# tensorlayer/HyperPose

Hardware: NVIDIA H100
Metric: frames/sec end-to-end (conv+PAF parse) OpenPose-COCO 368x656 (higher is better)
Workload: dtype f16 operands, f32 accumulate (conv); f32/f64 (parse)

## Files before the change

### hyperpose_b200/capi.py

```python
from __future__ import annotations

import ctypes as C
import os
import struct

import numpy as np

PKG = os.path.dirname(os.path.abspath(__file__))
LIB_PATH = os.path.join(PKG, "libhyperpose_b200.so")

N_PARTS, N_PAIRS = 18, 19
HP_OK, HP_ERR_ARG, HP_ERR_CAPACITY, HP_ERR_UNSUPPORTED, HP_ERR_CUDA, HP_ERR_BATCH = 0, -1, -2, -3, -4, -5

PART_DT = np.dtype({"names": ["has_value", "x", "y", "score"], "formats": ["<i4", "<f4", "<f4", "<f4"]})
HUMAN_DT = np.dtype([("parts", PART_DT, (N_PARTS,)), ("score", "<f4")])
PEAK_DT = np.dtype([("part_id", "<i4"), ("x", "<i4"), ("y", "<i4"), ("score", "<f4"), ("id", "<i4")])
CONN_DT = np.dtype([("cid1", "<i4"), ("cid2", "<i4"), ("score", "<f4")])
assert HUMAN_DT.itemsize == 292

EXPORTS = [
    "hp_last_error", "hp_device_count", "hp_version",
    "hp_paf_create", "hp_paf_destroy", "hp_paf_set_conf_thresh", "hp_paf_set_paf_thresh", "hp_paf_set_capacity",
    "hp_paf_process_host", "hp_paf_process_host_batched", "hp_paf_process_device", "hp_paf_fetch",
    "hp_paf_debug_peaks", "hp_paf_debug_connections", "hp_paf_launch_count", "hp_paf_copy_results_device", "hp_paf_debug_timing",
# ... 151 lines not shown
        _bind_engine(L)
        L._engine_bound = True
    check(L.hp_handoff_enable(1 if on else 0))


EXPORTS += [
    "hp_engine_create", "hp_engine_destroy", "hp_engine_info", "hp_engine_infer_u8_host", "hp_engine_infer_u8_device",
    "hp_engine_infer_f32_host", "hp_engine_outputs", "hp_engine_read_outputs_host", "hp_engine_copy_outputs_device", "hp_engine_sync",
    "hp_engine_launch_count", "hp_engine_debug_read_buffer", "hp_engine_debug_write_buffer", "hp_engine_debug_run_ops",
    "hp_pose_run_u8_host", "hp_engine_stage_frame_u8", "hp_engine_infer_staged", "hp_engine_debug_read_frames", "hp_engine_set_output_override", "hp_engine_set_profiling", "hp_engine_get_profile",
    "hp_engine_read_outputs_frames", "hp_engine_head_type", "hp_handoff_enable", "hp_handoff_stats",
    "hp_pose_submit_u8_host", "hp_pose_collect", "hp_pose_stats", "hp_paf_prepare", "hp_paf_state", "hp_paf_copy_results_host_async",
    "hp_paf_grow_capacity", "hp_pool_create", "hp_pool_destroy", "hp_pool_size", "hp_pool_set_capacity", "hp_pool_run_u8_host",
    "hp_pool_set_output_override", "hp_pool_launch_count", "hp_default_device", "hp_handoff_device_of",
    "hp_engine_create_ex", "hp_engine_dtype", "hp_pose_submit_u8_device", "hp_engine_debug_op_kernel",
    "hp_engine_debug_op_epilogue",
    "hp_engine_calibrate_u8", "hp_pack_int8_calibrated",
]


def _bind_engine(L):
    vp, ip = C.c_void_p, C.POINTER(C.c_int)
    L.hp_engine_create.argtypes = [C.POINTER(vp), vp, C.c_size_t, C.c_int, C.c_int, C.c_int, C.c_double, C.c_int, C.c_int]
    L.hp_engine_create_ex.argtypes = [C.POINTER(vp), vp, C.c_size_t, C.c_int, C.c_int, C.c_int, C.c_double, C.c_int, C.c_int, C.c_int]
    L.hp_engine_dtype.argtypes = [vp]
    L.hp_engine_destroy.argtypes = [vp]
    L.hp_engine_destroy.restype = None
    L.hp_engine_info.argtypes = [vp, ip, ip, ip, ip, ip, ip, ip, C.POINTER(C.c_double)]
    L.hp_engine_infer_u8_host.argtypes = [vp, vp, C.c_int]
    L.hp_engine_infer_u8_device.argtypes = [vp, vp, C.c_int, vp]
    L.hp_engine_infer_f32_host.argtypes = [vp, vp, C.c_int]
    L.hp_engine_outputs.argtypes = [vp, C.POINTER(vp), C.POINTER(vp), C.POINTER(vp)]
    L.hp_engine_read_outputs_host.argtypes = [vp, vp, vp, C.c_int]
    L.hp_engine_sync.argtypes = [vp]
    L.hp_engine_copy_outputs_device.argtypes = [vp, vp, vp, C.c_int, vp]
    L.hp_engine_launch_count.argtypes = [vp]
    L.hp_engine_launch_count.restype = C.c_longlong
    L.hp_engine_debug_read_buffer.argtypes = [vp, C.c_int, vp, C.c_int, ip, ip, ip]
    L.hp_engine_debug_write_buffer.argtypes = [vp, C.c_int, vp, C.c_int]
    L.hp_engine_debug_run_ops.argtypes = [vp, C.c_int, C.c_int, C.c_int]
    L.hp_engine_debug_op_kernel.argtypes = [vp, C.c_int, C.c_char_p, C.c_int]
    L.hp_engine_debug_op_epilogue.argtypes = [vp, C.c_int, ip]
    L.hp_engine_calibrate_u8.argtypes = [vp, vp, C.c_int, vp, C.c_int]
    L.hp_pack_int8_calibrated.argtypes = [vp, C.c_size_t]
    L.hp_pose_run_u8_host.argtypes = [vp, vp, vp, C.c_int, vp, C.c_int, ip]
    L.hp_engine_stage_frame_u8.argtypes = [vp, C.c_int, vp, C.c_int, C.c_int, C.c_int]
    L.hp_engine_infer_staged.argtypes = [vp, C.c_int]
    L.hp_engine_debug_read_frames.argtypes = [vp, vp, C.c_int]
    L.hp_engine_set_output_override.argtypes = [vp, vp, vp]
    L.hp_engine_set_profiling.argtypes = [vp, C.c_int]
    L.hp_engine_get_profile.argtypes = [vp, vp, vp, vp, C.c_int, ip, C.POINTER(C.c_longlong)]
    L.hp_engine_read_outputs_frames.argtypes = [vp, C.POINTER(vp), C.POINTER(vp), C.c_int, C.c_int]
    L.hp_engine_head_type.argtypes = [vp]
    L.hp_handoff_enable.argtypes = [C.c_int]
    L.hp_handoff_stats.argtypes = [C.POINTER(C.c_longlong)] * 4
    L.hp_pose_submit_u8_host.argtypes = [vp, vp, vp, C.c_int, ip]
    L.hp_pose_submit_u8_device.argtypes = [vp, vp, vp, C.c_int, ip]
# ... 143 lines not shown
        return out

    def debug_run_ops(self, first: int, last: int, n: int):
        check(lib().hp_engine_debug_run_ops(self._h, first, last, n))

    def debug_op_kernel(self, op: int) -> str:
        buf = C.create_string_buffer(64)
        check(lib().hp_engine_debug_op_kernel(self._h, op, buf, len(buf)))
        return buf.value.decode()

    def debug_op_epilogue(self, op: int) -> str:
        v = C.c_int(0)
        check(lib().hp_engine_debug_op_epilogue(self._h, op, C.byref(v)))
        return "tma" if v.value else "reg"

    def set_output_override(self, d_conf_ptr: int, d_paf_ptr: int):
        check(lib().hp_engine_set_output_override(self._h, d_conf_ptr, d_paf_ptr))

    def set_profiling(self, enable: bool):
        check(lib().hp_engine_set_profiling(self._h, 1 if enable else 0))

    def get_profile(self):
        cap = 1024
        ms = np.zeros(cap, np.float64); ty = np.zeros(cap, np.int32); fl = np.zeros(cap, np.float64)
        n, runs = C.c_int(), C.c_longlong()
        check(lib().hp_engine_get_profile(self._h, ms.ctypes.data, ty.ctypes.data, fl.ctypes.data, cap, C.byref(n), C.byref(runs)))
        return ms[:n.value], ty[:n.value], fl[:n.value], runs.value

    def run_pose(self, parser: "PafParser", frames: np.ndarray, cap: int = 128):
        frames = np.ascontiguousarray(frames, np.uint8)
# ... 242 lines not shown
```

### hyperpose_b200/csrc/conv_wgmma.cuh

```cuda
#pragma once
#include <cuda.h>
#include <cuda_fp16.h>
#include <cuda_runtime.h>
#include <stdint.h>

#include <type_traits>

namespace hpb {

constexpr int CONV_BLOCK_M = 128;
constexpr int CONV_BLOCK_K = 64;
constexpr int TF32_BLOCK_K = 32;
constexpr int CONV_MAX_STAGES = 8;
constexpr int CONV_THREADS = 384;
constexpr int CONV_A_BYTES = CONV_BLOCK_M * 128;
constexpr size_t CONV_SMEM_LIMIT = 227 * 1024;

enum ConvOutMode : int {
    OUT_F16_NHWC = 0,
    OUT_F32_NCHW_SPLIT = 1,
};

struct ConvParams {
    int Nb, H, W;
// ... 694 lines not shown
__device__ __forceinline__ uint64_t make_sw128_kmajor_desc_at(uint32_t smem_addr, uint32_t sbo)
{
    uint64_t d = 0;
    d |= (uint64_t)((smem_addr & 0x3ffffu) >> 4);
    d |= (uint64_t)1 << 16;
    d |= (uint64_t)((sbo >> 4) & 0x3fffu) << 32;
    d |= (uint64_t)1 << 62;
    return d;
}
template <uint32_t N> __device__ __forceinline__ void setmaxnreg_dec() { asm volatile("setmaxnreg.dec.sync.aligned.u32 %0;" ::"n"(N)); }
template <uint32_t N> __device__ __forceinline__ void setmaxnreg_inc() { asm volatile("setmaxnreg.inc.sync.aligned.u32 %0;" ::"n"(N)); }
__device__ __forceinline__ void stmatrix_x4(uint32_t addr, uint32_t r0, uint32_t r1, uint32_t r2, uint32_t r3)
{
    asm volatile("stmatrix.sync.aligned.m8n8.x4.shared.b16 [%0], {%1, %2, %3, %4};" ::"r"(addr), "r"(r0), "r"(r1), "r"(r2), "r"(r3) : "memory");
}
__device__ __forceinline__ void st_shared_u32(uint32_t addr, uint32_t v) { asm volatile("st.shared.b32 [%0], %1;" ::"r"(addr), "r"(v) : "memory"); }
__device__ __forceinline__ void named_barrier_sync(int id, int threads) { asm volatile("bar.sync %0, %1;" ::"r"(id), "r"(threads) : "memory"); }
__device__ __forceinline__ void tma_store_4d(const CUtensorMap* m, uint32_t src, int c0, int c1, int c2, int c3)
{
    asm volatile("cp.async.bulk.tensor.4d.global.shared::cta.bulk_group [%0, {%2, %3, %4, %5}], [%1];"
                 ::"l"(m), "r"(src), "r"(c0), "r"(c1), "r"(c2), "r"(c3) : "memory");
}
__device__ __forceinline__ void bulk_commit() { asm volatile("cp.async.bulk.commit_group;" ::: "memory"); }
template <int N> __device__ __forceinline__ void bulk_wait_read() { asm volatile("cp.async.bulk.wait_group.read %0;" ::"n"(N) : "memory"); }
template <int N> __device__ __forceinline__ void bulk_wait() { asm volatile("cp.async.bulk.wait_group %0;" ::"n"(N) : "memory"); }
__device__ __forceinline__ uint32_t half2_bits(__half2 h) { return *reinterpret_cast<uint32_t*>(&h); }
}

template <int BN, bool kPool, int kBlocks>
__device__ __forceinline__ void halo_epilogue(const float (&acc)[kBlocks][BN / 2], const HaloParams& p, int n, int y0, int x0, int g, int n0,
                                              int row_base, int warp, int lane)
// ... 119 lines not shown
                }
            }
        }
        ptx::fence_proxy_async();
        ptx::named_barrier_sync(bar_id, 128);
        if (leader) {
            const int x = kPool ? x0 >> 1 : x0, y = kPool ? (y0 + ty0) >> 1 : y0 + ty0;
            ptx::tma_store_4d(tmap_o, slot, och, x, y, n);
            if (BN == 128 && n0 + 64 < p.cout_g)
                ptx::tma_store_4d(tmap_o, slot + (uint32_t)kSliceBytes, och + 64, x, y, n);
            ptx::bulk_commit();
        }
    }
}

template <int BN, int kBlocks>
__device__ __forceinline__ void halo_kstep(float (&acc)[kBlocks][BN / 2], uint32_t abase, int r, int s, int BW, uint32_t sbo, const uint8_t* s_b,
                                           uint64_t* b_full, RingPos b, int c_or_tap HALO_PH_PARAM)
{
    uint64_t da[kBlocks];
#pragma unroll
    for (int m = 0; m < kBlocks; ++m) da[m] = ptx::make_sw128_kmajor_desc_at(abase + (uint32_t)(((m * 8 + r) * BW + s) * 128), sbo);
    const uint64_t db = ptx::make_sw128_kmajor_desc(ptx::smem_u32(s_b + (size_t)b.slot * BN * 128));
    HALO_TIMED(HALO_PH_B_WAIT, ptx::mbar_wait(ptx::smem_u32(b_full + b.slot), b.phase));
#pragma unroll
    for (int m = 0; m < kBlocks; ++m) ptx::fence_acc(acc[m]);
    ptx::wgmma_fence();
#pragma unroll
    for (int k = 0; k < 4; ++k)
#pragma unroll
// ... 14 lines not shown
        if (tma) {
            if constexpr (kItem != HaloItem::Wide)
                halo_epilogue_tma<BN, kPool, kShape.blocks, kShape.stage_slots, true>(acc, p, tmap_o, stage, n, y0, x0, g, n0, row_base, warp, lane,
                                                                                     leader HALO_PH_ARG);
            else if (p.box_bytes >= kShape.blocks * BN * 128)
                halo_epilogue_tma<BN, kPool, kShape.blocks, kShape.blocks, false>(acc, p, tmap_o, stage, n, y0, x0, g, n0, row_base, warp, lane,
                                                                                 leader HALO_PH_ARG);
            else
                halo_epilogue_tma<BN, kPool, kShape.blocks, 1, true>(acc, p, tmap_o, stage, n, y0, x0, g, n0, row_base, warp, lane, leader HALO_PH_ARG);
            return;
        }
    }
    halo_epilogue<BN, kPool, kShape.blocks>(acc, p, n, y0, x0, g, n0, row_base, warp, lane);
}

template <int BN, bool kPool, HaloItem kItem>
__global__ void __launch_bounds__(CONV_THREADS, 1)
conv_halo_kernel(const __grid_constant__ CUtensorMap tmap_x, const __grid_constant__ CUtensorMap tmap_b, const __grid_constant__ CUtensorMap tmap_o,
                 const HaloParams p)
{
    static_assert(!(kItem == HaloItem::Wide && kPool), "the pooled epilogue pairs pixel rows of one m64 block; it has no wide form");
    static_assert(kItem != HaloItem::PingPong || BN == 64 || BN == 128, "the ping-pong item is built for the VGG trunk's widths, BN = 64 and 128");
    constexpr HaloShape kShape = halo_shape(kItem, BN);
    constexpr int B_BYTES = BN * 128;
    constexpr bool kTmaForm = BN % 64 == 0;
    extern __shared__ uint8_t smem_raw[];
    ptx::pdl_launch_dependents();
    uint8_t* smem = (uint8_t*)(((uintptr_t)smem_raw + 1023) & ~(uintptr_t)1023);
    uint8_t* s_box = smem;
    uint8_t* s_b = s_box + (size_t)kShape.box_slots * kShape.tiles * p.box_bytes;
    uint8_t* s_stage = s_b + (size_t)p.num_stages * B_BYTES;
    uint64_t* a_full = (uint64_t*)(s_stage + 2 * (size_t)p.stage_bytes);
    uint64_t* a_empty = a_full + kShape.box_slots;
    uint64_t* b_full = a_empty + kShape.box_slots;
    uint64_t* b_empty = b_full + CONV_MAX_STAGES;
    uint64_t* turn = b_empty + CONV_MAX_STAGES;

    const int wg = threadIdx.x >> 7, warp = threadIdx.x >> 5, lane = threadIdx.x & 31;
    const int n_tiles_g = p.cout_g_pad / BN;
    const int nt_total = p.groups * n_tiles_g;
    const int sp_per_img = p.tiles_x * p.tiles_y;
    const int total_items = (p.Nb * sp_per_img + kShape.tiles - 1) / kShape.tiles * nt_total;
    const int chunks = p.cin_g / CONV_BLOCK_K;
    const int taps = p.R * p.S;
    const int BW = HALO_TW + p.S - 1, BH = HALO_TH + p.R - 1;

    if (threadIdx.x == 0) {
        ptx::prefetch_tmap(&tmap_x);
        ptx::prefetch_tmap(&tmap_b);
        if (kTmaForm && p.tma_store) ptx::prefetch_tmap(&tmap_o);
        for (int i = 0; i < kShape.box_slots; ++i) {
            ptx::mbar_init(ptx::smem_u32(a_full + i), 1);
            ptx::mbar_init(ptx::smem_u32(a_empty + i), kShape.slot_warps);
        }
        for (int i = 0; i < p.num_stages; ++i) {
            ptx::mbar_init(ptx::smem_u32(b_full + i), 1);
            ptx::mbar_init(ptx::smem_u32(b_empty + i), kShape.slot_warps);
        }
        if constexpr (kItem == HaloItem::PingPong) {
            ptx::mbar_init(ptx::smem_u32(turn), 4);
            ptx::mbar_init(ptx::smem_u32(turn + 1), 4);
        }
        ptx::fence_barrier_init();
    }
    __syncthreads();
    ptx::pdl_wait();

    auto decode = [&](int item, int& sp, int& g, int& n0) {
        const int nt = item % nt_total;
        sp = item / nt_total * kShape.tiles;
        g = nt / n_tiles_g;
        n0 = (nt - g * n_tiles_g) * BN;
    };
    auto tile_pos = [&](int sp, int& n, int& y0, int& x0) {
        n = sp / sp_per_img;
        const int t = sp - n * sp_per_img;
        const int ty = t / p.tiles_x;
        y0 = ty * HALO_TH;
// ... 11 lines not shown
            const int pad_h = p.R / 2, pad_w = p.S / 2;
            for (int item = blockIdx.x; item < total_items; item += gridDim.x) {
                int sp, g, n0;
                decode(item, sp, g, n0);
                for (int c = 0; c < chunks; ++c) {
                    ptx::mbar_wait(ptx::smem_u32(a_empty + a.slot), a.phase ^ 1);
                    const uint32_t fa = ptx::smem_u32(a_full + a.slot);
                    ptx::mbar_expect_tx(fa, (uint32_t)(kShape.tiles * BH * BW * 128));
#pragma unroll
                    for (int t = 0; t < kShape.tiles; ++t) {
                        int n, y0, x0;
                        tile_pos(sp + t, n, y0, x0);
                        ptx::tma_load_4d(ptx::smem_u32(s_box + (size_t)(a.slot * kShape.tiles + t) * p.box_bytes), &tmap_x, fa,
                                         p.in_ch_off + g * p.cin_g + c * CONV_BLOCK_K, x0 - pad_w, y0 - pad_h, n);
                    }
                    a.step(kShape.box_slots);
                    for (int tap = 0; tap < taps; ++tap) {
                        ptx::mbar_wait(ptx::smem_u32(b_empty + b.slot), b.phase ^ 1);
                        const uint32_t fb = ptx::smem_u32(b_full + b.slot);
                        ptx::mbar_expect_tx(fb, (uint32_t)B_BYTES);
                        ptx::tma_load_2d(ptx::smem_u32(s_b + (size_t)b.slot * B_BYTES), &tmap_b, fb, tap * p.cin_g + c * CONV_BLOCK_K, g * p.cout_g_pad + n0);
                        b.step(p.num_stages);
                    }
                }
            }
        }
        return;
    }

    if constexpr (kShape.move_regs) ptx::setmaxnreg_inc<HALO_WIDE_CONSUMER_REGS>();
    const int half = wg - 1;
    const uint32_t sbo = (uint32_t)BW * 128u;
    const bool tma = kTmaForm && p.tma_store;
    const bool leader = (threadIdx.x & 127) == 0;
    const uint32_t stage = ptx::smem_u32(s_stage + (size_t)half * p.stage_bytes);
    float acc[kShape.blocks][BN / 2];
    if constexpr (kItem == HaloItem::PingPong) {
        const int item_stages = chunks * taps;
        if (half) {
            a.advance(chunks, kShape.box_slots);
            b.advance(item_stages, p.num_stages);
        }
        for (int j = half, item = blockIdx.x + half * gridDim.x; item < total_items; j += 2, item += 2 * gridDim.x) {
            int sp, g, n0;
            decode(item, sp, g, n0);
            if (j > 0) HALO_TIMED(HALO_PH_TURN_WAIT, ptx::mbar_wait(ptx::smem_u32(turn + half), (uint32_t)((j - 1) >> 1) & 1u));
            int prev_st = 0, prev_bs = 0;
            for (int c = 0; c < chunks; ++c) {
                HALO_TIMED(HALO_PH_A_WAIT, ptx::mbar_wait(ptx::smem_u32(a_full + a.slot), a.phase));
                const uint32_t abase = ptx::smem_u32(s_box + (size_t)a.slot * p.box_bytes);
                for (int tap = 0; tap < taps; ++tap) {
                    const int r = tap / p.S, s = tap - r * p.S;
// ... 74 lines not shown
            const int last = (a.slot + kShape.box_slots - 1) % kShape.box_slots;
            const uint32_t dst = kItem == HaloItem::Wide ? ptx::smem_u32(s_box + (size_t)(last * kShape.tiles + box) * p.box_bytes) : stage;
            halo_store<BN, kPool, kItem>(acc, p, &tmap_o, tma, dst, n, y0, x0, g, n0, row_base, warp, lane, leader HALO_PH_ARG);
            HALO_PH_ADD(HALO_PH_EPILOGUE, t_epi);
        }
    }
    if (tma && leader) ptx::bulk_wait<0>();
#ifdef HPB_HALO_PHASES
    HALO_PH_ADD(HALO_PH_TOTAL, t_start);
    if ((threadIdx.x & 127) == 0)
        for (int i = 0; i < HALO_PH_COUNT; ++i) atomicAdd(g_halo_phases + i, (unsigned long long)ph[i]);
#endif
}

inline int halo_box_bytes(int R, int S) { return ((HALO_TH + R - 1) * (HALO_TW + S - 1) * 128 + 1023) & ~1023; }
inline size_t conv_halo_smem_bytes(int R, int S, int BN, int stages, HaloItem it, bool tma_store)
{
    const HaloShape sh = halo_shape(it, BN);
    return 1024 + (size_t)sh.box_slots * sh.tiles * halo_box_bytes(R, S) + (size_t)stages * BN * 128 +
           (tma_store ? 2 * (size_t)halo_stage_bytes(BN, it) : 0) + (2 * sh.box_slots + 2 * CONV_MAX_STAGES + 2) * 8;
}
inline int conv_halo_pick_stages(int R, int S, int BN, HaloItem it, bool tma_store)
{
    int s = CONV_MAX_STAGES;
    while (s > 2 && conv_halo_smem_bytes(R, S, BN, s, it, tma_store) > CONV_SMEM_LIMIT) --s;
    return s;
}

}
```

### hyperpose_b200/csrc/engine.cu

```cuda
#include <cuda.h>
#include <cuda_fp16.h>
#include <cuda_runtime.h>
#include <math.h>
#include <stdint.h>
#include <stdlib.h>
#include <string.h>

#include <algorithm>
#include <memory>
#include <string>
#include <vector>

#include "../../include/hyperpose_b200.h"
#include "common.h"
#include "conv_wgmma.cuh"
#include "helpers_tf32_int8.cuh"
#include "handoff.h"
#include "pair_math.cuh"
#include "pack_format.h"

namespace {
using namespace hpb;


// ... 506 lines not shown
    for (int bn : { 96, 64 })
        if (round_up(cout_g, bn) < round_up(cout_g, best)) best = bn;
    return best;
}

struct ConvPlan {
    ConvParams prm;
    CUtensorMap tmap_a, tmap_b;
    CUtensorMap tmap_x;
    CUtensorMap tmap_o;
    void* d_w = nullptr;
    bool monotone_act = false;
    HaloParams hp;
    HaloItem halo_item = HaloItem::Narrow;
    bool halo_pool = false;
    float* d_bias = nullptr;
    float* d_alpha = nullptr;
    float* d_mul = nullptr;
    size_t smem = 0;
    double flops_per_frame = 0;
};

enum class Launch : uint8_t {
    None,
    Im2col,
    StemOrIm2col,
    Conv,
    ConvStem,
    Halo,
    DwTma,
// ... 132 lines not shown
inline float tf32_round(float x)
{
    uint32_t u;
    memcpy(&u, &x, 4);
    if ((u & 0x7f800000u) != 0x7f800000u) u = (u + 0x1000u) & 0xffffe000u;
    memcpy(&x, &u, 4);
    return x;
}

bool halo_tma_store_ok(const HaloParams& h, int BN)
{
    return BN % 64 == 0 && h.out_ld % 8 == 0 && h.out_ch_off % 8 == 0 && (h.groups * h.cout_g) % 8 == 0 &&
           (h.groups == 1 || h.cout_g % BN == 0);
}

int set_halo_item(const hp_engine* e, EngOp& op, HaloItem item, bool pool)
{
    HaloParams& h = op.plan.hp;
    const int BN = op.plan.prm.BN;
    h.tma_store = e->opt.halo_tma_store && halo_tma_store_ok(h, BN);
    h.stage_bytes = h.tma_store ? halo_stage_bytes(BN, item) : 0;
    h.num_stages = conv_halo_pick_stages(h.R, h.S, BN, item, h.tma_store);
    op.plan.smem = conv_halo_smem_bytes(h.R, h.S, BN, h.num_stages, item, h.tma_store);
    op.plan.halo_item = item;
    op.plan.halo_pool = pool;
    op.launch = Launch::Halo;
    if (!h.tma_store) return HP_OK;
    const int oh = pool ? h.H / 2 : h.H, ow = pool ? h.W / 2 : h.W, box = pool ? HALO_TW / 2 : HALO_TW;
    return make_tmap_act_box(&op.plan.tmap_o, h.out, e->max_batch, oh, ow, h.out_ch_off + h.groups * h.cout_g, h.out_ld, box, box,
                             CU_TENSOR_MAP_SWIZZLE_128B);
}

bool halo_wide_faster(int R, long wide_items, int sms)
{
    return R == 7 && wide_items >= sms;
}

bool halo_pp_exists(int R, int BN) { return R == 3 && (BN == 64 || BN == 128); }
bool halo_pp_faster(int chunks, bool pooled, long items, int sms) { return (chunks >= 4 || pooled) && items >= 2L * sms; }
// ... 174 lines not shown
}

template <typename T, bool kRes, int kStemR = 0>
const void* conv_kernel_bn(int BN)
{
    switch (BN) {
    case 16: return (const void*)conv_wgmma_kernel<T, 16, kRes, kStemR>;
    case 32: return (const void*)conv_wgmma_kernel<T, 32, kRes, kStemR>;
    case 48: return (const void*)conv_wgmma_kernel<T, 48, kRes, kStemR>;
    case 64: return (const void*)conv_wgmma_kernel<T, 64, kRes, kStemR>;
    case 96: return (const void*)conv_wgmma_kernel<T, 96, kRes, kStemR>;
    case 128: return (const void*)conv_wgmma_kernel<T, 128, kRes, kStemR>;
    }
    return nullptr;
}
const void* halo_kernel(int BN, HaloItem item, bool pool)
{
    using I = HaloItem;
    if (item == I::Wide) return BN == 128 && !pool ? (const void*)conv_halo_kernel<128, false, I::Wide> : nullptr;
    if (item == I::PingPong) {
        if (BN == 64) return pool ? (const void*)conv_halo_kernel<64, true, I::PingPong> : (const void*)conv_halo_kernel<64, false, I::PingPong>;
        if (BN == 128) return pool ? (const void*)conv_halo_kernel<128, true, I::PingPong> : (const void*)conv_halo_kernel<128, false, I::PingPong>;
        return nullptr;
    }
    switch (BN) {
    case 16: return pool ? (const void*)conv_halo_kernel<16, true, I::Narrow> : (const void*)conv_halo_kernel<16, false, I::Narrow>;
    case 32: return pool ? (const void*)conv_halo_kernel<32, true, I::Narrow> : (const void*)conv_halo_kernel<32, false, I::Narrow>;
    case 48: return pool ? (const void*)conv_halo_kernel<48, true, I::Narrow> : (const void*)conv_halo_kernel<48, false, I::Narrow>;
    case 64: return pool ? (const void*)conv_halo_kernel<64, true, I::Narrow> : (const void*)conv_halo_kernel<64, false, I::Narrow>;
    case 96: return pool ? (const void*)conv_halo_kernel<96, true, I::Narrow> : (const void*)conv_halo_kernel<96, false, I::Narrow>;
    case 128: return pool ? (const void*)conv_halo_kernel<128, true, I::Narrow> : (const void*)conv_halo_kernel<128, false, I::Narrow>;
    }
    return nullptr;
}
// ... 28 lines not shown
int launch_conv(hp_engine* e, EngOp& op, int N, cudaStream_t st, bool u8_input)
{
    ConvPlan& pl = op.plan;
    ConvParams p = pl.prm;
    p.Nb = N;
    const int stem_R = op.launch == Launch::ConvStem && u8_input ? (int)op.po.R : 0;
    p.frames = e->cur_frames ? e->cur_frames : e->d_frames;
    if (op.launch == Launch::Halo) {
        HaloParams h = pl.hp;
        h.Nb = N;
        const int tiles = halo_shape(pl.halo_item, p.BN).tiles;
        const long items = ((long)N * h.tiles_x * h.tiles_y + tiles - 1) / tiles * h.groups * (h.cout_g_pad / p.BN);
        cudaLaunchAttribute at[1];
        const cudaLaunchConfig_t cfg = pdl_config((int)std::min<long>(e->num_sms - e->reserve_sms, items), CONV_THREADS, pl.smem, st, at);
        void* args[] = { (void*)&pl.tmap_x, (void*)&pl.tmap_b, (void*)&pl.tmap_o, (void*)&h };
        HP_CUDA_TRY(cudaLaunchKernelExC(&cfg, halo_kernel(p.BN, pl.halo_item, pl.halo_pool), args));
        return HP_OK;
    }
    p.m_tiles = (int)(((size_t)N * p.H * p.W + CONV_BLOCK_M - 1) / CONV_BLOCK_M);
    const int n_tiles = p.m_tiles * p.groups * (p.cout_g_pad / p.BN);
    const int grid = std::min(e->num_sms - e->reserve_sms, n_tiles);
    cudaLaunchAttribute at[1];
    const cudaLaunchConfig_t cfg = pdl_config(grid, CONV_THREADS, pl.smem, st, at);
    void* args[] = { (void*)&pl.tmap_a, (void*)&pl.tmap_b, (void*)&p };
    HP_CUDA_TRY(cudaLaunchKernelExC(&cfg, conv_kernel(e->dtype, p.res_mode != 0, p.BN, stem_R), args));
    return HP_OK;
}

bool collect_one(hp_engine* e, bool blocking)
{
    if (e->ev_tail >= e->ev_head) return false;
// ... 569 lines not shown
        if (a.launch != Launch::DwTma || b.launch != Launch::DwTma || a.po.in_buf != b.po.in_buf || a.po.in_ch_off != b.po.in_ch_off ||
            a.po.cout_g != b.po.cout_g || a.po.out_buf != b.po.out_buf || dw_dilation(a.po) != 1 || dw_dilation(b.po) != 1) continue;
        a.launch = Launch::DwTmaPair;
        b.launch = Launch::None;
    }
    int launches = 0;
    for (const EngOp& o : e->ops) {
        if ((o.po.type == OP_CONV || o.po.type == OP_DWCONV || o.po.type == OP_MAXPOOL2) && o.launch != Launch::None) ++launches;
        e->step_kernels += kernels_launched(o.launch, true);
    }
    const double per_launch = launches ? e->flops_per_frame * e->max_batch / launches : 0.0;
    e->use_pdl = dtype == HP_DTYPE_F16 && launches > 0 && per_launch < 10e9;
    for (const EngOp& o : e->ops) {
        if (o.po.type != OP_CONV) continue;
        if (o.launch == Launch::Halo &&
            cudaFuncSetAttribute(halo_kernel(o.plan.prm.BN, o.plan.halo_item, o.plan.halo_pool), cudaFuncAttributeMaxDynamicSharedMemorySize, (int)max_smem) != cudaSuccess) {
            set_error("engine: cannot opt in to %zu bytes of dynamic shared memory (halo)", max_smem);
            return fail(HP_ERR_CUDA);
        }
        const int stem_R = o.launch == Launch::ConvStem ? (int)o.po.R : 0;
        for (int v = 0; v < 3; ++v)
            if ((v < 2 || stem_R) &&
                cudaFuncSetAttribute(conv_kernel(dtype, v == 1, o.plan.prm.BN, v == 2 ? stem_R : 0), cudaFuncAttributeMaxDynamicSharedMemorySize, (int)max_smem) != cudaSuccess) {
                set_error("engine: cannot opt in to %zu bytes of dynamic shared memory", max_smem);
                return fail(HP_ERR_CUDA);
            }
    }
    if (cudaDeviceSynchronize() != cudaSuccess) { set_error("hp_engine_create: device error during set-up: %s", cudaGetErrorString(cudaGetLastError())); return fail(HP_ERR_CUDA); }
    *out = e;
    return HP_OK;
}
// ... 341 lines not shown
        s = s.back() == '>' ? s.substr(0, s.size() - 1) + "," + d + ">" : s + "<" + d + ">";
    }
    if ((int)s.size() >= cap) { set_error("hp_engine_debug_op_kernel: %zu-character name, capacity %d", s.size(), cap); return HP_ERR_CAPACITY; }
    memcpy(name, s.c_str(), s.size() + 1);
    return HP_OK;
}

int hp_engine_debug_op_epilogue(const hp_engine* e, int op, int* tma_store)
{
    if (!e || op < 0 || op >= (int)e->ops.size() || !tma_store) { set_error("hp_engine_debug_op_epilogue: bad argument"); return HP_ERR_ARG; }
    const EngOp& o = e->ops[op];
    *tma_store = o.launch == Launch::Halo && o.plan.hp.tma_store ? 1 : 0;
    return HP_OK;
}

long long hp_engine_launch_count(const hp_engine* e) { return e ? e->launches : 0; }

int hp_engine_set_output_override(hp_engine* e, const float* d_conf, const float* d_paf)
{
    if (!e) return HP_ERR_ARG;
    e->override_conf = d_conf;
    e->override_paf = d_paf;
    return HP_OK;
}

int hp_engine_set_profiling(hp_engine* e, int enable)
{
    if (!e) return HP_ERR_ARG;
    HP_CUDA_TRY(cudaSetDevice(e->device));
    if (enable && e->ev.empty()) {
// ... 326 lines not shown
```

### include/hyperpose_b200.h

```cpp
#ifndef HYPERPOSE_B200_H
#define HYPERPOSE_B200_H

#include <stddef.h>
#include <stdint.h>

#ifdef __cplusplus
extern "C" {
#endif

#define HP_N_PARTS 18
#define HP_N_PAIRS 19

typedef enum hp_status {
    HP_OK = 0,
    HP_ERR_ARG = -1,
    HP_ERR_CAPACITY = -2,
    HP_ERR_UNSUPPORTED = -3,
    HP_ERR_CUDA = -4,
    HP_ERR_BATCH = -5
} hp_status;

typedef struct hp_body_part {
    int32_t has_value;
    float x, y, score;
// ... 90 lines not shown
int hp_engine_infer_f32_host(hp_engine* e, const float* nchw, int N);
int hp_engine_outputs(hp_engine* e, const float** d_conf, const float** d_paf, void** stream);
int hp_engine_read_outputs_host(hp_engine* e, float* conf, float* paf, int N);
int hp_engine_read_outputs_frames(hp_engine* e, float* const* conf_frames, float* const* paf_frames, int N, int publish);
int hp_engine_head_type(const hp_engine* e);
int hp_handoff_enable(int on);
int hp_handoff_stats(long long* published, long long* hits, long long* batch_parses, long long* misses);
int hp_engine_copy_outputs_device(hp_engine* e, float* d_conf, float* d_paf, int N, void* stream);
int hp_engine_sync(hp_engine* e);
long long hp_engine_launch_count(const hp_engine* e);
int hp_engine_debug_read_buffer(hp_engine* e, int buf, void* out_f16, int N, int* H, int* W, int* C);
int hp_engine_debug_write_buffer(hp_engine* e, int buf, const void* in_f16, int N);
int hp_engine_debug_run_ops(hp_engine* e, int first_op, int last_op, int N);
int hp_engine_debug_op_kernel(const hp_engine* e, int op, char* name, int cap);
int hp_engine_debug_op_epilogue(const hp_engine* e, int op, int* tma_store);

int hp_engine_set_output_override(hp_engine* e, const float* d_conf, const float* d_paf);
int hp_engine_set_profiling(hp_engine* e, int enable);
int hp_engine_get_profile(hp_engine* e, double* ms_per_op, int* op_type, double* flops_per_op, int cap, int* n_ops, long long* runs);

int hp_pose_run_u8_host(hp_engine* e, hp_paf* parser, const uint8_t* frames, int N, hp_human* out, int cap, int* n_out);
int hp_pose_submit_u8_host(hp_engine* e, hp_paf* parser, const uint8_t* frames, int N, int* ticket);
int hp_pose_submit_u8_device(hp_engine* e, hp_paf* parser, const uint8_t* d_frames, int N, int* ticket);
int hp_pose_collect(hp_engine* e, int ticket, hp_human* out, int cap, int* n_out);
int hp_pose_stats(const hp_engine* e, long long* graph_captures, long long* graph_launches);
int hp_pose_submit_pifpaf_u8_host(hp_engine* e, hp_pifpaf* decoder, const uint8_t* frames, int N, int* ticket);
int hp_pose_submit_pifpaf_u8_device(hp_engine* e, hp_pifpaf* decoder, const uint8_t* d_frames, int N, int* ticket);
int hp_pifpaf_pipeline_info(hp_pifpaf* p, void** stream, void** inputs_free_event, int* hcap);
int hp_pifpaf_copy_results_host_async(hp_pifpaf* p, hp_human* pin_humans, int* pin_counts_flags, int N, void* stream);
int hp_pifpaf_grow_capacity(hp_pifpaf* p, int flags);
// ... 22 lines not shown
```

Baseline: 1024.

## Keep 3x3 conv weights resident in shared memory for the 64-channel ping-pong halo kernel

For 3x3, 64-in/64-out, ungrouped convs using the ping-pong halo item, all nine weight tap tiles are loaded into shared memory once per CTA. The per-item B-tile streaming loop and its full/empty barriers are removed, and the freed smem is spent on extra input box slots. The MMA computes with weights as the A operand, giving a channel-major accumulator. A new epilogue writes it with transposed stmatrix (or a pooled u16 scatter) before the TMA store. This cuts redundant weight TMA traffic and producer synchronisation on the early VGG layers, at the cost of a new epilogue layout path that may be less efficient or carry indexing bugs.

Measured after the change: 1055 (median of 6 runs). 3.0% higher.

```diff
diff --git a/hyperpose_b200/capi.py b/hyperpose_b200/capi.py
--- a/hyperpose_b200/capi.py
+++ b/hyperpose_b200/capi.py
@@ -189,7 +189,7 @@
     "hp_paf_grow_capacity", "hp_pool_create", "hp_pool_destroy", "hp_pool_size", "hp_pool_set_capacity", "hp_pool_run_u8_host",
     "hp_pool_set_output_override", "hp_pool_launch_count", "hp_default_device", "hp_handoff_device_of",
     "hp_engine_create_ex", "hp_engine_dtype", "hp_pose_submit_u8_device", "hp_engine_debug_op_kernel",
-    "hp_engine_debug_op_epilogue",
+    "hp_engine_debug_op_epilogue", "hp_engine_debug_op_weights",
     "hp_engine_calibrate_u8", "hp_pack_int8_calibrated",
 ]
 
@@ -216,6 +216,7 @@
     L.hp_engine_debug_run_ops.argtypes = [vp, C.c_int, C.c_int, C.c_int]
     L.hp_engine_debug_op_kernel.argtypes = [vp, C.c_int, C.c_char_p, C.c_int]
     L.hp_engine_debug_op_epilogue.argtypes = [vp, C.c_int, ip]
+    L.hp_engine_debug_op_weights.argtypes = [vp, C.c_int, ip]
     L.hp_engine_calibrate_u8.argtypes = [vp, vp, C.c_int, vp, C.c_int]
     L.hp_pack_int8_calibrated.argtypes = [vp, C.c_size_t]
     L.hp_pose_run_u8_host.argtypes = [vp, vp, vp, C.c_int, vp, C.c_int, ip]
@@ -389,6 +390,11 @@
         check(lib().hp_engine_debug_op_epilogue(self._h, op, C.byref(v)))
         return "tma" if v.value else "reg"
 
+    def debug_op_weights(self, op: int) -> str:
+        v = C.c_int(0)
+        check(lib().hp_engine_debug_op_weights(self._h, op, C.byref(v)))
+        return "resident" if v.value else "streamed"
+
     def set_output_override(self, d_conf_ptr: int, d_paf_ptr: int):
         check(lib().hp_engine_set_output_override(self._h, d_conf_ptr, d_paf_ptr))
 
diff --git a/hyperpose_b200/csrc/conv_wgmma.cuh b/hyperpose_b200/csrc/conv_wgmma.cuh
--- a/hyperpose_b200/csrc/conv_wgmma.cuh
+++ b/hyperpose_b200/csrc/conv_wgmma.cuh
@@ -732,7 +732,12 @@
 {
     asm volatile("stmatrix.sync.aligned.m8n8.x4.shared.b16 [%0], {%1, %2, %3, %4};" ::"r"(addr), "r"(r0), "r"(r1), "r"(r2), "r"(r3) : "memory");
 }
+__device__ __forceinline__ void stmatrix_x4_trans(uint32_t addr, uint32_t r0, uint32_t r1, uint32_t r2, uint32_t r3)
+{
+    asm volatile("stmatrix.sync.aligned.m8n8.x4.trans.shared.b16 [%0], {%1, %2, %3, %4};" ::"r"(addr), "r"(r0), "r"(r1), "r"(r2), "r"(r3) : "memory");
+}
 __device__ __forceinline__ void st_shared_u32(uint32_t addr, uint32_t v) { asm volatile("st.shared.b32 [%0], %1;" ::"r"(addr), "r"(v) : "memory"); }
+__device__ __forceinline__ void st_shared_u16(uint32_t addr, unsigned short v) { asm volatile("st.shared.b16 [%0], %1;" ::"r"(addr), "h"(v) : "memory"); }
 __device__ __forceinline__ void named_barrier_sync(int id, int threads) { asm volatile("bar.sync %0, %1;" ::"r"(id), "r"(threads) : "memory"); }
 __device__ __forceinline__ void tma_store_4d(const CUtensorMap* m, uint32_t src, int c0, int c1, int c2, int c3)
 {
@@ -882,6 +887,63 @@
     }
 }
 
+template <bool kPool>
+__device__ __forceinline__ void halo_epilogue_tma_cm(const float (&acc)[64], const HaloParams& p, const CUtensorMap* tmap_o, uint32_t stage,
+                                                     int n, int y0, int x0, int warp, int lane, bool leader HALO_PH_PARAM)
+{
+    constexpr int kSliceBytes = (kPool ? 16 : 64) * 128;
+    const int c = 16 * (warp & 3) + (lane >> 2);
+    const float b[2] = { __ldg(p.bias + c), __ldg(p.bias + c + 8) }, a[2] = { __ldg(p.alpha + c), __ldg(p.alpha + c + 8) };
+    const int bar_id = warp >> 2;
+#pragma unroll
+    for (int m = 0; m < 2; ++m) {
+        const uint32_t slot = stage + (uint32_t)(m * kSliceBytes);
+        HALO_PH_MARK(t_wait);
+        if (leader) ptx::bulk_wait_read<1>();
+        ptx::named_barrier_sync(bar_id, 128);
+#ifdef HPB_HALO_PHASES
+        { const long long d = clock64() - t_wait; ph[HALO_PH_STAGE_WAIT] += d; ph[HALO_PH_EPILOGUE] -= d; }
+#endif
+        if constexpr (kPool) {
+#pragma unroll
+            for (int pr = 0; pr < 4; ++pr) {
+                const int y = 8 * m + 2 * pr, q = 4 * pr + (lane & 3);
+#pragma unroll
+                for (int h = 0; h < 2; ++h) {
+                    const float v0 = fmaxf(acc[4 * y + 2 * h], acc[4 * y + 4 + 2 * h]), v1 = fmaxf(acc[4 * y + 2 * h + 1], acc[4 * y + 4 + 2 * h + 1]);
+                    float v = fmaxf(v0, v1) + b[h];
+                    v = v > 0.f ? v : v * a[h];
+                    ptx::st_shared_u16(slot + (uint32_t)(q * 128 + ((((c >> 3) + h) ^ (q & 7)) << 4) + (c & 7) * 2),
+                                       __half_as_ushort(__float2half_rn(v)));
+                }
+            }
+        } else {
+            const int r = lane & 7, i = lane >> 3;
+#pragma unroll
+            for (int jp = 0; jp < 4; ++jp) {
+                uint32_t v[4];
+#pragma unroll
+                for (int k = 0; k < 4; ++k) {
+                    const int y = 8 * m + 2 * jp + (k >> 1), h = k & 1;
+                    float a0 = acc[4 * y + 2 * h] + b[h], a1 = acc[4 * y + 2 * h + 1] + b[h];
+                    a0 = a0 > 0.f ? a0 : a0 * a[h];
+                    a1 = a1 > 0.f ? a1 : a1 * a[h];
+                    v[k] = ptx::half2_bits(__floats2half2_rn(a0, a1));
+                }
+                const int q = (2 * jp + (i >> 1)) * 8 + r, j = 2 * (warp & 3) + (i & 1);
+                ptx::stmatrix_x4_trans(slot + (uint32_t)(q * 128 + ((j ^ r) << 4)), v[0], v[1], v[2], v[3]);
+            }
+        }
+        ptx::fence_proxy_async();
+        ptx::named_barrier_sync(bar_id, 128);
+        if (leader) {
+            const int x = kPool ? x0 >> 1 : x0, y = kPool ? (y0 + 8 * m) >> 1 : y0 + 8 * m;
+            ptx::tma_store_4d(tmap_o, slot, p.out_ch_off, x, y, n);
+            ptx::bulk_commit();
+        }
+    }
+}
+
 template <int BN, int kBlocks>
 __device__ __forceinline__ void halo_kstep(float (&acc)[kBlocks][BN / 2], uint32_t abase, int r, int s, int BW, uint32_t sbo, const uint8_t* s_b,
                                            uint64_t* b_full, RingPos b, int c_or_tap HALO_PH_PARAM)
@@ -926,25 +988,28 @@
     halo_epilogue<BN, kPool, kShape.blocks>(acc, p, n, y0, x0, g, n0, row_base, warp, lane);
 }
 
-template <int BN, bool kPool, HaloItem kItem>
+template <int BN, bool kPool, HaloItem kItem, bool kResident = false>
 __global__ void __launch_bounds__(CONV_THREADS, 1)
 conv_halo_kernel(const __grid_constant__ CUtensorMap tmap_x, const __grid_constant__ CUtensorMap tmap_b, const __grid_constant__ CUtensorMap tmap_o,
                  const HaloParams p)
 {
     static_assert(!(kItem == HaloItem::Wide && kPool), "the pooled epilogue pairs pixel rows of one m64 block; it has no wide form");
     static_assert(kItem != HaloItem::PingPong || BN == 64 || BN == 128, "the ping-pong item is built for the VGG trunk's widths, BN = 64 and 128");
+    static_assert(!kResident || (kItem == HaloItem::PingPong && BN == 64), "resident weights: the ping-pong item at BN = 64");
     constexpr HaloShape kShape = halo_shape(kItem, BN);
     constexpr int B_BYTES = BN * 128;
     constexpr bool kTmaForm = BN % 64 == 0;
+    const int taps = p.R * p.S;
+    const int box_slots = kResident ? p.num_stages : kShape.box_slots, b_tiles = kResident ? taps : p.num_stages;
     extern __shared__ uint8_t smem_raw[];
     ptx::pdl_launch_dependents();
     uint8_t* smem = (uint8_t*)(((uintptr_t)smem_raw + 1023) & ~(uintptr_t)1023);
     uint8_t* s_box = smem;
-    uint8_t* s_b = s_box + (size_t)kShape.box_slots * kShape.tiles * p.box_bytes;
-    uint8_t* s_stage = s_b + (size_t)p.num_stages * B_BYTES;
+    uint8_t* s_b = s_box + (size_t)box_slots * kShape.tiles * p.box_bytes;
+    uint8_t* s_stage = s_b + (size_t)b_tiles * B_BYTES;
     uint64_t* a_full = (uint64_t*)(s_stage + 2 * (size_t)p.stage_bytes);
-    uint64_t* a_empty = a_full + kShape.box_slots;
-    uint64_t* b_full = a_empty + kShape.box_slots;
+    uint64_t* a_empty = a_full + box_slots;
+    uint64_t* b_full = a_empty + box_slots;
     uint64_t* b_empty = b_full + CONV_MAX_STAGES;
     uint64_t* turn = b_empty + CONV_MAX_STAGES;
 
@@ -954,18 +1019,17 @@
     const int sp_per_img = p.tiles_x * p.tiles_y;
     const int total_items = (p.Nb * sp_per_img + kShape.tiles - 1) / kShape.tiles * nt_total;
     const int chunks = p.cin_g / CONV_BLOCK_K;
-    const int taps = p.R * p.S;
     const int BW = HALO_TW + p.S - 1, BH = HALO_TH + p.R - 1;
 
     if (threadIdx.x == 0) {
         ptx::prefetch_tmap(&tmap_x);
         ptx::prefetch_tmap(&tmap_b);
         if (kTmaForm && p.tma_store) ptx::prefetch_tmap(&tmap_o);
-        for (int i = 0; i < kShape.box_slots; ++i) {
+        for (int i = 0; i < box_slots; ++i) {
             ptx::mbar_init(ptx::smem_u32(a_full + i), 1);
             ptx::mbar_init(ptx::smem_u32(a_empty + i), kShape.slot_warps);
         }
-        for (int i = 0; i < p.num_stages; ++i) {
+        for (int i = 0; i < (kResident ? 1 : p.num_stages); ++i) {
             ptx::mbar_init(ptx::smem_u32(b_full + i), 1);
             ptx::mbar_init(ptx::smem_u32(b_empty + i), kShape.slot_warps);
         }
@@ -974,6 +1038,11 @@
             ptx::mbar_init(ptx::smem_u32(turn + 1), 4);
         }
         ptx::fence_barrier_init();
+        if constexpr (kResident) {
+            const uint32_t fb = ptx::smem_u32(b_full);
+            ptx::mbar_expect_tx(fb, (uint32_t)(taps * B_BYTES));
+            for (int tap = 0; tap < taps; ++tap) ptx::tma_load_2d(ptx::smem_u32(s_b + (size_t)tap * B_BYTES), &tmap_b, fb, tap * p.cin_g, 0);
+        }
     }
     __syncthreads();
     ptx::pdl_wait();
@@ -1015,14 +1084,15 @@
                         ptx::tma_load_4d(ptx::smem_u32(s_box + (size_t)(a.slot * kShape.tiles + t) * p.box_bytes), &tmap_x, fa,
                                          p.in_ch_off + g * p.cin_g + c * CONV_BLOCK_K, x0 - pad_w, y0 - pad_h, n);
                     }
-                    a.step(kShape.box_slots);
-                    for (int tap = 0; tap < taps; ++tap) {
-                        ptx::mbar_wait(ptx::smem_u32(b_empty + b.slot), b.phase ^ 1);
-                        const uint32_t fb = ptx::smem_u32(b_full + b.slot);
-                        ptx::mbar_expect_tx(fb, (uint32_t)B_BYTES);
-                        ptx::tma_load_2d(ptx::smem_u32(s_b + (size_t)b.slot * B_BYTES), &tmap_b, fb, tap * p.cin_g + c * CONV_BLOCK_K, g * p.cout_g_pad + n0);
-                        b.step(p.num_stages);
-                    }
+                    a.step(box_slots);
+                    if constexpr (!kResident)
+                        for (int tap = 0; tap < taps; ++tap) {
+                            ptx::mbar_wait(ptx::smem_u32(b_empty + b.slot), b.phase ^ 1);
+                            const uint32_t fb = ptx::smem_u32(b_full + b.slot);
+                            ptx::mbar_expect_tx(fb, (uint32_t)B_BYTES);
+                            ptx::tma_load_2d(ptx::smem_u32(s_b + (size_t)b.slot * B_BYTES), &tmap_b, fb, tap * p.cin_g + c * CONV_BLOCK_K, g * p.cout_g_pad + n0);
+                            b.step(p.num_stages);
+                        }
                 }
             }
         }
@@ -1036,7 +1106,42 @@
     const bool leader = (threadIdx.x & 127) == 0;
     const uint32_t stage = ptx::smem_u32(s_stage + (size_t)half * p.stage_bytes);
     float acc[kShape.blocks][BN / 2];
-    if constexpr (kItem == HaloItem::PingPong) {
+    if constexpr (kResident) {
+        float cm[64];
+        const uint32_t sw = ptx::smem_u32(s_b);
+        if (half) a.step(box_slots);
+        HALO_TIMED(HALO_PH_B_WAIT, ptx::mbar_wait(ptx::smem_u32(b_full), 0));
+        for (int j = half, item = blockIdx.x + half * gridDim.x; item < total_items; j += 2, item += 2 * gridDim.x) {
+            if (j > 0) HALO_TIMED(HALO_PH_TURN_WAIT, ptx::mbar_wait(ptx::smem_u32(turn + half), (uint32_t)((j - 1) >> 1) & 1u));
+            HALO_TIMED(HALO_PH_A_WAIT, ptx::mbar_wait(ptx::smem_u32(a_full + a.slot), a.phase));
+            const uint32_t abase = ptx::smem_u32(s_box + (size_t)a.slot * p.box_bytes);
+            ptx::fence_acc(cm);
+            ptx::wgmma_fence();
+#pragma unroll
+            for (int r = 0; r < 3; ++r)
+#pragma unroll
+                for (int s = 0; s < 3; ++s) {
+                    const uint64_t dw = ptx::make_sw128_kmajor_desc(sw + (uint32_t)((r * 3 + s) * B_BYTES));
+                    const uint64_t dx = ptx::make_sw128_kmajor_desc_at(abase + (uint32_t)((r * BW + s) * 128), sbo);
+#pragma unroll
+                    for (int k = 0; k < 4; ++k)
+                        ptx::wgmma<__half, 128>(cm, dw + (uint64_t)(k * 2), dx + (uint64_t)(k * 2), (r | s | k) != 0 ? 1u : 0u);
+                }
+            ptx::wgmma_commit();
+            ptx::fence_acc(cm);
+            if (lane == 0) ptx::mbar_arrive(ptx::smem_u32(turn + (half ^ 1)));
+            HALO_TIMED(HALO_PH_MMA_WAIT, ptx::wgmma_wait<0>());
+            ptx::fence_acc(cm);
+            if (lane == 0) ptx::mbar_arrive(ptx::smem_u32(a_empty + a.slot));
+            a.step(box_slots);
+            a.step(box_slots);
+            HALO_PH_MARK(t_epi);
+            int n, y0, x0;
+            tile_pos(item / nt_total, n, y0, x0);
+            halo_epilogue_tma_cm<kPool>(cm, p, &tmap_o, stage, n, y0, x0, warp, lane, leader HALO_PH_ARG);
+            HALO_PH_ADD(HALO_PH_EPILOGUE, t_epi);
+        }
+    } else if constexpr (kItem == HaloItem::PingPong) {
         const int item_stages = chunks * taps;
         if (half) {
             a.advance(chunks, kShape.box_slots);
@@ -1141,16 +1246,17 @@
 }
 
 inline int halo_box_bytes(int R, int S) { return ((HALO_TH + R - 1) * (HALO_TW + S - 1) * 128 + 1023) & ~1023; }
-inline size_t conv_halo_smem_bytes(int R, int S, int BN, int stages, HaloItem it, bool tma_store)
+inline size_t conv_halo_smem_bytes(int R, int S, int BN, int stages, HaloItem it, bool tma_store, bool resident = false)
 {
     const HaloShape sh = halo_shape(it, BN);
-    return 1024 + (size_t)sh.box_slots * sh.tiles * halo_box_bytes(R, S) + (size_t)stages * BN * 128 +
-           (tma_store ? 2 * (size_t)halo_stage_bytes(BN, it) : 0) + (2 * sh.box_slots + 2 * CONV_MAX_STAGES + 2) * 8;
-}
-inline int conv_halo_pick_stages(int R, int S, int BN, HaloItem it, bool tma_store)
+    const int box_slots = resident ? stages : sh.box_slots, b_tiles = resident ? R * S : stages;
+    return 1024 + (size_t)box_slots * sh.tiles * halo_box_bytes(R, S) + (size_t)b_tiles * BN * 128 +
+           (tma_store ? 2 * (size_t)halo_stage_bytes(BN, it) : 0) + (2 * box_slots + 2 * CONV_MAX_STAGES + 2) * 8;
+}
+inline int conv_halo_pick_stages(int R, int S, int BN, HaloItem it, bool tma_store, bool resident = false)
 {
     int s = CONV_MAX_STAGES;
-    while (s > 2 && conv_halo_smem_bytes(R, S, BN, s, it, tma_store) > CONV_SMEM_LIMIT) --s;
+    while (s > 2 && conv_halo_smem_bytes(R, S, BN, s, it, tma_store, resident) > CONV_SMEM_LIMIT) --s;
     return s;
 }
 
diff --git a/hyperpose_b200/csrc/engine.cu b/hyperpose_b200/csrc/engine.cu
--- a/hyperpose_b200/csrc/engine.cu
+++ b/hyperpose_b200/csrc/engine.cu
@@ -544,6 +544,7 @@
     HaloParams hp;
     HaloItem halo_item = HaloItem::Narrow;
     bool halo_pool = false;
+    bool halo_resident = false;
     float* d_bias = nullptr;
     float* d_alpha = nullptr;
     float* d_mul = nullptr;
@@ -706,15 +707,23 @@
            (h.groups == 1 || h.cout_g % BN == 0);
 }
 
+bool halo_resident_ok(const HaloParams& h, int BN, HaloItem item)
+{
+    return item == HaloItem::PingPong && BN == 64 && h.R == 3 && h.S == 3 && h.groups == 1 && h.cout_g_pad == BN && h.cin_g == CONV_BLOCK_K && h.tma_store &&
+           conv_halo_smem_bytes(h.R, h.S, BN, 4, item, true, true) <= CONV_SMEM_LIMIT;
+}
+
 int set_halo_item(const hp_engine* e, EngOp& op, HaloItem item, bool pool)
 {
     HaloParams& h = op.plan.hp;
     const int BN = op.plan.prm.BN;
     h.tma_store = e->opt.halo_tma_store && halo_tma_store_ok(h, BN);
     h.stage_bytes = h.tma_store ? halo_stage_bytes(BN, item) : 0;
-    h.num_stages = conv_halo_pick_stages(h.R, h.S, BN, item, h.tma_store);
-    op.plan.smem = conv_halo_smem_bytes(h.R, h.S, BN, h.num_stages, item, h.tma_store);
+    const bool resident = halo_resident_ok(h, BN, item);
+    h.num_stages = conv_halo_pick_stages(h.R, h.S, BN, item, h.tma_store, resident);
+    op.plan.smem = conv_halo_smem_bytes(h.R, h.S, BN, h.num_stages, item, h.tma_store, resident);
     op.plan.halo_item = item;
+    op.plan.halo_resident = resident;
     op.plan.halo_pool = pool;
     op.launch = Launch::Halo;
     if (!h.tma_store) return HP_OK;
@@ -919,10 +928,14 @@
     }
     return nullptr;
 }
-const void* halo_kernel(int BN, HaloItem item, bool pool)
+const void* halo_kernel(int BN, HaloItem item, bool pool, bool resident)
 {
     using I = HaloItem;
     if (item == I::Wide) return BN == 128 && !pool ? (const void*)conv_halo_kernel<128, false, I::Wide> : nullptr;
+    if (resident)
+        return item != I::PingPong || BN != 64 ? nullptr
+               : pool                          ? (const void*)conv_halo_kernel<64, true, I::PingPong, true>
+                                               : (const void*)conv_halo_kernel<64, false, I::PingPong, true>;
     if (item == I::PingPong) {
         if (BN == 64) return pool ? (const void*)conv_halo_kernel<64, true, I::PingPong> : (const void*)conv_halo_kernel<64, false, I::PingPong>;
         if (BN == 128) return pool ? (const void*)conv_halo_kernel<128, true, I::PingPong> : (const void*)conv_halo_kernel<128, false, I::PingPong>;
@@ -981,7 +994,7 @@
         cudaLaunchAttribute at[1];
         const cudaLaunchConfig_t cfg = pdl_config((int)std::min<long>(e->num_sms - e->reserve_sms, items), CONV_THREADS, pl.smem, st, at);
         void* args[] = { (void*)&pl.tmap_x, (void*)&pl.tmap_b, (void*)&pl.tmap_o, (void*)&h };
-        HP_CUDA_TRY(cudaLaunchKernelExC(&cfg, halo_kernel(p.BN, pl.halo_item, pl.halo_pool), args));
+        HP_CUDA_TRY(cudaLaunchKernelExC(&cfg, halo_kernel(p.BN, pl.halo_item, pl.halo_pool, pl.halo_resident), args));
         return HP_OK;
     }
     p.m_tiles = (int)(((size_t)N * p.H * p.W + CONV_BLOCK_M - 1) / CONV_BLOCK_M);
@@ -1581,7 +1594,7 @@
     for (const EngOp& o : e->ops) {
         if (o.po.type != OP_CONV) continue;
         if (o.launch == Launch::Halo &&
-            cudaFuncSetAttribute(halo_kernel(o.plan.prm.BN, o.plan.halo_item, o.plan.halo_pool), cudaFuncAttributeMaxDynamicSharedMemorySize, (int)max_smem) != cudaSuccess) {
+            cudaFuncSetAttribute(halo_kernel(o.plan.prm.BN, o.plan.halo_item, o.plan.halo_pool, o.plan.halo_resident), cudaFuncAttributeMaxDynamicSharedMemorySize, (int)max_smem) != cudaSuccess) {
             set_error("engine: cannot opt in to %zu bytes of dynamic shared memory (halo)", max_smem);
             return fail(HP_ERR_CUDA);
         }
@@ -1953,6 +1966,14 @@
     return HP_OK;
 }
 
+int hp_engine_debug_op_weights(const hp_engine* e, int op, int* resident)
+{
+    if (!e || op < 0 || op >= (int)e->ops.size() || !resident) { set_error("hp_engine_debug_op_weights: bad argument"); return HP_ERR_ARG; }
+    const EngOp& o = e->ops[op];
+    *resident = o.launch == Launch::Halo && o.plan.halo_resident ? 1 : 0;
+    return HP_OK;
+}
+
 long long hp_engine_launch_count(const hp_engine* e) { return e ? e->launches : 0; }
 
 int hp_engine_set_output_override(hp_engine* e, const float* d_conf, const float* d_paf)
diff --git a/include/hyperpose_b200.h b/include/hyperpose_b200.h
--- a/include/hyperpose_b200.h
+++ b/include/hyperpose_b200.h
@@ -128,6 +128,7 @@
 int hp_engine_debug_run_ops(hp_engine* e, int first_op, int last_op, int N);
 int hp_engine_debug_op_kernel(const hp_engine* e, int op, char* name, int cap);
 int hp_engine_debug_op_epilogue(const hp_engine* e, int op, int* tma_store);
+int hp_engine_debug_op_weights(const hp_engine* e, int op, int* resident);
 
 int hp_engine_set_output_override(hp_engine* e, const float* d_conf, const float* d_paf);
 int hp_engine_set_profiling(hp_engine* e, int enable);
```
